# zkemail/zk-email-verify

Measured on NVIDIA H100. Metric: EmailVerifier proofs/sec (witness+prove), higher is better.
Workload: dtype u256 (BN254 Fr/Fq integers, 8x32-bit limbs)

## Files before the change

### zk-email-verify_b200/csrc/engine.cu

```cuda
#include "ff.cuh"
namespace zke { namespace dev { unsigned long long g_kernel_launches = 0; } }
#include "witness.cu"
#include "matvec.cu"
#include "ntt.cu"
#include "msm.cuh"
#include "fixed_base.cuh"
namespace zke { namespace dev {
ZKE_DEFINE_CONSTANT_UPLOAD(upload_constants_engine)
cudaError_t upload_constants_msm_g1(const FieldConsts*, const FieldConsts*);
cudaError_t upload_constants_msm_g2(const FieldConsts*, const FieldConsts*);
cudaError_t upload_constants_fixed_base(const FieldConsts*, const FieldConsts*);
cudaError_t upload_constants_verify(const FieldConsts*, const FieldConsts*);
cudaError_t upload_constants_registry(const FieldConsts*, const FieldConsts*);
} }

#include "../../include/zkemail_b200.h"
#include "cuda_host.hpp"
#include "engine.hpp"
#include "witness_program.hpp"
#include "binfile.hpp"
#include "ec_host.hpp"
#include "setup_host.hpp"
#include <algorithm>
#include <cstdio>
#include <cstring>
#include <atomic>
#include <memory>
#include <mutex>
#include <thread>
#include <unordered_map>

using namespace zke;

void zke::select_device(int device) {
    int n = 0;
    if (cudaGetDeviceCount(&n) != cudaSuccess || n == 0) throw std::runtime_error("no CUDA device available (this library has no CPU fallback)");
    if (device < 0 || device >= n) throw std::runtime_error("bad device index");
    CUDA_OK(cudaSetDevice(device));
    dev::FieldConsts fr, fq;
    fill_consts(fr, fr_params());
    fill_consts(fq, fq_params());
    CUDA_OK(dev::upload_constants_engine(&fr, &fq));
    CUDA_OK(dev::upload_constants_msm_g1(&fr, &fq));
    CUDA_OK(dev::upload_constants_msm_g2(&fr, &fq));
    CUDA_OK(dev::upload_constants_fixed_base(&fr, &fq));
    CUDA_OK(dev::upload_constants_verify(&fr, &fq));
    CUDA_OK(dev::upload_constants_registry(&fr, &fq));
    CUDA_OK(dev::configure_witness_kernel());
}

namespace {

template <class F>
std::vector<AffineH<F>> window_table(const AffineH<F>& gen) {
    std::vector<AffineH<F>> t(32 * 256, AffineH<F>::inf());
    JacobianH<F> base = JacobianH<F>::from_affine(gen);
    for (int w = 0; w < 32; ++w) {
        JacobianH<F> acc = JacobianH<F>::inf();
        for (int d = 1; d < 256; ++d) {
            acc = acc.add(base);
            t[w * 256 + d] = acc.to_affine();
        }
        for (int k = 0; k < 8; ++k) base = base.dbl();
    }
    return t;
}

std::vector<U256> to_standard(const std::vector<Fr>& v) {
    std::vector<U256> out(v.size());
    const unsigned T = std::max(1u, std::min(16u, std::thread::hardware_concurrency()));
    std::vector<std::thread> th;
    for (unsigned t = 0; t < T; ++t)
        th.emplace_back([&, t]() { for (size_t i = v.size() * t / T; i < v.size() * (t + 1) / T; ++i) out[i] = v[i].to_u256(); });
    for (auto& x : th) x.join();
    return out;
}

}

struct zke_zkey {
    uint32_t n_vars = 0, n_public = 0, log_n = 0;
    int device = 0;
    bool toy = false;
    bool delta_one = false;
    G1AffineH alpha1, beta1, delta1;
    G2AffineH beta2, gamma2, delta2;
    std::vector<G1AffineH> ic;
    DevBuf A, B1, B2, C, H;
    int h_levels = 1;
    dev::MsmConfig cfg_h;
    bool has_coefs = false;
    std::vector<uint32_t> a_ptr, a_var, a_coef, b_ptr, b_var, b_coef;
    std::vector<U256> coefs;
};

struct zke_ctx {
    const zke_circuit* circuit = nullptr;
    const zke_zkey* zkey = nullptr;
    int device = 0;
    uint32_t max_batch = 0;
    uint32_t n_vars = 0, n_public = 0, n_inputs = 0;
    cudaStream_t stream = nullptr;
    DevBuf ops, iter_hdr, lc_terms, aux, coop, coef_r, small_inv;
    std::vector<uint32_t> coef_word;
    std::vector<uint32_t> iter_info;
    DevBuf a_ptr, a_terms, b_ptr, b_terms, c_ptr, c_terms;
    dev::DevProgram prog;
    dev::DevR1cs r1cs;
    DevBuf tw_fwd, tw_inv, coset_scale;
    dev::NttTables ntt;
    size_t stride = 0;
    DevBuf inputs, check_flag;
    uint32_t inputs_resident = 0;
    struct Slot {
        bool allocated = false, busy = false;
        DevBuf w_all, inputs, results, first_bad;
        uint8_t* results_host = nullptr;
        uint8_t* publics_host = nullptr;
        std::vector<cudaEvent_t> done;
        cudaEvent_t witness_done = nullptr;
        uint32_t loaded = 0;
        uint32_t batch = 0;
        std::vector<uint8_t> rs;
    };
    Slot slots[2];
    uint64_t n_submitted = 0, n_collected = 0;
    int shard_rank = -1, shard_world = 0, shard_log_g = 0, shard_stage = 0;
    struct Lane { cudaStream_t st = nullptr, heavy = nullptr; cudaEvent_t ev[6] = {}; DevBuf va, vb, vc, vd, msm_ws; };
    Lane lanes[ZKE_MAX_LANES];
    int n_lanes = 1, lanes_alloc = 0;
    int finish_threads = 4;
    dev::MsmConfig cfg_w, cfg_h;
    bool split_streams = true;
    std::vector<uint32_t> bad_host;
    bool profile = false;
    std::vector<cudaEvent_t> ev_pool;
    size_t ev_used = 0;
    struct Span { int stage; size_t e0, e1; };
    std::vector<Span> spans;
    double stage_ms[ZKE_N_STAGES] = {0};
    uint64_t stage_count[ZKE_N_STAGES] = {0};
    cudaEvent_t ev(size_t* idx) {
        if (ev_used == ev_pool.size()) { cudaEvent_t e; cudaEventCreate(&e); ev_pool.push_back(e); }
        *idx = ev_used;
        return ev_pool[ev_used++];
    }
    size_t mark(cudaStream_t st) { size_t i; cudaEventRecord(ev(&i), st); return i; }
    size_t mark() { return mark(stream); }
    void collect() {
        for (auto& s : spans) {
            float ms = 0;
            if (cudaEventElapsedTime(&ms, ev_pool[s.e0], ev_pool[s.e1]) == cudaSuccess) { stage_ms[s.stage] += ms; stage_count[s.stage]++; }
        }
        spans.clear();
        ev_used = 0;
    }
};

static const uint32_t SETUP_SLAB = 1u << 20;
static void h_table_config(zke_zkey* zk, size_t N) {
    const char* e = getenv("ZKE_H_PRECOMP");
    const bool precomp = !(e && atoi(e) == 0);
    zk->cfg_h = dev::msm_config_full((uint32_t)N, precomp);
    zk->h_levels = precomp ? dev::msm_windows(zk->cfg_h) : 1;
}
static void build_h_levels(zke_zkey* zk, size_t N, uint8_t* scratch, cudaStream_t st) {
    for (int lvl = 1; lvl < zk->h_levels; ++lvl) {
        const uint8_t* prev = zk->H.p + (size_t)(lvl - 1) * N * sizeof(dev::G1Affine);
        uint8_t* cur = zk->H.p + (size_t)lvl * N * sizeof(dev::G1Affine);
        for (size_t off = 0; off < N; off += SETUP_SLAB) {
            uint32_t cnt = (uint32_t)std::min<size_t>(SETUP_SLAB, N - off);
            dev::scale_pow2_batch<dev::Fq>(prev + sizeof(dev::G1Affine) * off, cnt, zk->cfg_h.c, scratch, cur + sizeof(dev::G1Affine) * off, st);
        }
    }
    CHECK_LAUNCH();
    CUDA_OK(cudaStreamSynchronize(st));
}

static zke_zkey* do_setup(const zke_circuit* zc, uint64_t seed, int device) {
    select_device(device);
    const Circuit& c = zc->c;
    SetupScalars S = compute_setup_scalars(c, seed);
    std::unique_ptr<zke_zkey> zk(new zke_zkey());
    zk->n_vars = c.n_vars; zk->n_public = c.n_public(); zk->log_n = S.log_n; zk->device = device;
    zk->toy = true;
    const size_t N = (size_t)1 << S.log_n;
    const uint32_t m = c.n_vars, l = c.n_public();

    G1JacH g1 = G1JacH::from_affine(g1_generator());
    G2JacH g2 = G2JacH::from_affine(g2_generator());
    zk->alpha1 = g1.mul(S.alpha.to_u256()).to_affine();
    zk->beta1 = g1.mul(S.beta.to_u256()).to_affine();
    zk->delta1 = g1.mul(S.delta.to_u256()).to_affine();
    zk->beta2 = g2.mul(S.beta.to_u256()).to_affine();
    zk->gamma2 = g2.mul(S.gamma.to_u256()).to_affine();
    zk->delta2 = g2.mul(S.delta.to_u256()).to_affine();

    DevBuf t1, t2, scal, scratch;
    t1.upload(window_table<Fq>(g1_generator()));
    t2.upload(window_table<Fq2>(g2_generator()));
    const uint32_t SLAB = SETUP_SLAB;
// ... 479 lines not shown
    x->n_vars = cp ? cp->n_vars : zk->n_vars;
    x->n_public = cp ? cp->n_public() : zk->n_public;
    x->n_inputs = cp ? cp->n_inputs() : 0;
    int prio_least = 0, prio_greatest = 0;
    CUDA_OK(cudaDeviceGetStreamPriorityRange(&prio_least, &prio_greatest));
    CUDA_OK(cudaStreamCreateWithPriority(&x->stream, cudaStreamNonBlocking, prio_greatest));

    const std::vector<U256>& coefs = cp ? cp->coefs : zk->coefs;
    x->coef_word = coef_words(coefs);
    {
        std::vector<Fr> cr(std::max<size_t>(1, coefs.size()));
        for (size_t i = 0; i < coefs.size(); ++i) cr[i] = Fr::from_u256(coefs[i]);
        x->coef_r.upload(cr);
    }

    if (zk && cp && cp->r1cs_only && zk->has_coefs) check_key_matrices(*cp, *zk);

    if (cp && !cp->r1cs_only) upload_program(x.get(), *cp);
    upload_r1cs(x.get(), cp, zk);
    x->stride = (size_t)x->n_vars + (cp ? cp->n_temps : 0);
    x->inputs.alloc((size_t)std::max(1u, x->n_inputs) * 32 * max_batch);
    x->check_flag.alloc(8);
    x->bad_host.resize(max_batch);
    alloc_slot(x.get(), x->slots[0]);

    if (zk) {
        build_ntt_tables(x.get(), zk->log_n);
        open_lanes(x.get(), (size_t)1 << zk->log_n, prio_least, prio_greatest);
    }
    CUDA_OK(cudaDeviceSynchronize());
    return x.release();
}

static std::string assert_message(const zke_ctx* x, uint32_t email, uint32_t row) {
    std::string scope = "?";
    if (x->circuit) {
        const Circuit& c = x->circuit->c;
        if (row < c.scope_of_constraint.size()) scope = c.scopes[c.scope_of_constraint[row]];
    }
    return "Assert Failed: constraint " + std::to_string(row) + " in template " + scope + " @ email " + std::to_string(email);
}

static void require_idle(const zke_ctx* x) {
    if (x->n_submitted != x->n_collected) throw std::runtime_error("a submitted batch is still in flight: call zke_fullprove_collect first");
}

static void do_witness(zke_ctx* x, zke_ctx::Slot& S, const uint8_t* inputs, size_t batch) {
    if (!x->circuit) throw std::runtime_error("this context was opened from a .zkey alone: it has no witness program (use zke_load_witness / zke_wtns_prove)");
    const Circuit& c = x->circuit->c;
    if (c.r1cs_only) throw std::runtime_error(R1CS_NO_PROGRAM);
    if (batch == 0 || batch > x->max_batch) throw std::runtime_error("batch exceeds the context's max_batch");
    CUDA_OK(cudaSetDevice(x->device));
    const uint8_t* in_dev = x->inputs.p;
    if (inputs) {
        if (c.n_inputs()) CUDA_OK(cudaMemcpyAsync(S.inputs.p, inputs, (size_t)c.n_inputs() * 32 * batch, cudaMemcpyHostToDevice, x->stream));
        in_dev = S.inputs.p;
    } else if (x->inputs_resident < batch) {
        throw std::runtime_error("inputs == NULL but no (or too few) inputs are resident: call zke_upload_inputs first");
    }
    size_t p0 = 0;
    if (x->profile) p0 = x->mark();
    if (const char* tp = getenv("ZKE_WITNESS_TRACE")) {
        DevBuf tr;
        tr.alloc(8 * ((size_t)x->prog.n_iters + 1));
        dev::DevProgram P = x->prog;
        P.trace = (unsigned long long*)tr.p;
        dev::launch_witness(P, S.w_all.p, x->stride, in_dev, (uint32_t)batch, x->stream);
        CUDA_OK(cudaStreamSynchronize(x->stream));
        std::vector<unsigned long long> h(x->prog.n_iters);
        CUDA_OK(cudaMemcpy(h.data(), tr.p, 8 * h.size(), cudaMemcpyDeviceToHost));
        if (FILE* f = fopen(tp, "wb")) {
            fwrite(h.data(), 8, h.size(), f);
            fwrite(x->iter_info.data(), 4, x->iter_info.size(), f);
            fclose(f);
        }
    }
    dev::launch_witness(x->prog, S.w_all.p, x->stride, in_dev, (uint32_t)batch, x->stream);
    CHECK_LAUNCH();
    if (x->profile) x->spans.push_back({ZKE_STAGE_WITNESS, p0, x->mark()});
    S.loaded = (uint32_t)batch;
}

static int do_check(zke_ctx* x, zke_ctx::Slot& S, size_t batch, int32_t* status, std::string& msg) {
    CUDA_OK(cudaMemsetAsync(S.first_bad.p, 0xff, 4 * batch, x->stream));
    dev::launch_check_rows(x->r1cs, S.w_all.p, x->stride, (uint32_t)batch, (uint32_t*)S.first_bad.p, x->stream);
    CHECK_LAUNCH();
    CUDA_OK(cudaMemcpyAsync(x->bad_host.data(), S.first_bad.p, 4 * batch, cudaMemcpyDeviceToHost, x->stream));
    CUDA_OK(cudaStreamSynchronize(x->stream));
    if (x->profile) x->collect();
    int bad = 0;
    for (size_t e = 0; e < batch; ++e) {
        int32_t s = x->bad_host[e] == 0xffffffffu ? -1 : (int32_t)x->bad_host[e];
        if (status) status[e] = s;
        if (s >= 0) { if (!bad) msg = assert_message(x, (uint32_t)e, (uint32_t)s); ++bad; }
    }
    return bad;
}

static void write_fq(uint8_t* dst, const Fq& x) { U256 s = x.to_u256(); memcpy(dst, s.v, 32); }

template <class F>
static AffineH<F> finish_msm(const uint8_t* block, const dev::MsmConfig& cfg) {
    const XyzzH<F>* slots = reinterpret_cast<const XyzzH<F>*>(block);
    const int n_windows = cfg.precomputed ? 1 : (255 + cfg.c - 1) / cfg.c;
    XyzzH<F> acc = XyzzH<F>::inf();
    for (int j = n_windows - 1; j >= 0; --j) {
        if (!acc.is_inf()) for (int k = 0; k < cfg.c; ++k) acc.dbl();
        acc.add(slots[dev::MSM_ONES_SLOTS + j]);
    }
    if (cfg.classify) for (int i = 0; i < dev::MSM_ONES_SLOTS; ++i) acc.add(slots[i]);
    return acc.to_affine();
}

static void sync_lanes(zke_ctx* x) {
    cudaStreamSynchronize(x->stream);
    for (int i = 0; i < x->lanes_alloc; ++i) { cudaStreamSynchronize(x->lanes[i].st); cudaStreamSynchronize(x->lanes[i].heavy); }
}

static void enqueue_prove(zke_ctx* x, zke_ctx::Slot& S, size_t batch, const uint8_t* rs) {
    const zke_zkey* zk = x->zkey;
    if (!zk) throw std::runtime_error("context was opened without a proving key");
    if (batch == 0 || batch > S.loaded) throw std::runtime_error("no witness loaded for this batch (call zke_witness first)");
    if (rs) {
        for (size_t e = 0; e < 2 * batch; ++e) {
            U256 v;
            memcpy(v.v, rs + 32 * e, 32);
            if (u256_cmp(v, fr_params().p) >= 0) throw std::runtime_error("r / s not reduced mod the group order");
        }
        S.rs.assign(rs, rs + 64 * batch);
    } else {
        S.rs.clear();
    }
    CUDA_OK(cudaSetDevice(x->device));
    const uint32_t N = 1u << zk->log_n, m = x->n_vars, l = x->n_public;
    const bool prof = x->profile;
    const int n_lanes = prof ? 1 : x->n_lanes;
    if (const char* e = getenv("ZKE_SPLIT_STREAMS")) x->split_streams = atoi(e) != 0;
    if (l) CUDA_OK(cudaMemcpy2DAsync(S.publics_host, (size_t)l * 32, S.w_all.p + 32, x->stride * 32, (size_t)l * 32, batch, cudaMemcpyDeviceToHost, x->stream));
    CUDA_OK(cudaEventRecord(S.witness_done, x->stream));
    for (int i = 0; i < n_lanes; ++i) CUDA_OK(cudaStreamWaitEvent(x->lanes[i].st, S.witness_done, 0));
    for (size_t e = 0; e < batch; ++e) {
        zke_ctx::Lane& L = x->lanes[e % n_lanes];
        cudaStream_t st = L.st;
        const uint8_t* w = S.w_all.p + 32 * x->stride * e;
        uint8_t* res = S.results.p + (size_t)ZKE_RESULT_STRIDE * e;
        uint32_t* flag = (uint32_t*)(res + ZKE_RES_FLAG_OFF);
        size_t t0 = 0, t1 = 0;
        CUDA_OK(cudaMemsetAsync(flag, 0xff, 4, st));
        if (prof) t0 = x->mark(st);
        cudaStream_t hv = (prof || !x->split_streams) ? st : L.heavy;
        dev::launch_build_ab(x->r1cs, w, L.va.p, L.vb.p, L.vc.p, N, flag, st);
        if (prof) { t1 = x->mark(st); x->spans.push_back({ZKE_STAGE_MATVEC, t0, t1}); t0 = t1; }
        if (hv != st) { CUDA_OK(cudaEventRecord(L.ev[0], st)); CUDA_OK(cudaStreamWaitEvent(hv, L.ev[0], 0)); }
        dev::launch_intt_dif(L.va.p, x->ntt, x->coset_scale.p, hv);
        dev::launch_intt_dif(L.vb.p, x->ntt, x->coset_scale.p, hv);
        dev::launch_intt_dif(L.vc.p, x->ntt, x->coset_scale.p, hv);
        dev::launch_ntt_dit(L.va.p, x->ntt, hv);
        dev::launch_ntt_dit(L.vb.p, x->ntt, hv);
        dev::launch_ntt_dit(L.vc.p, x->ntt, hv);
        dev::launch_quotient(L.va.p, L.vb.p, L.vc.p, L.vd.p, N, hv);
        CHECK_LAUNCH();
        if (hv != st) CUDA_OK(cudaEventRecord(L.ev[1], hv));
        if (prof) { t1 = x->mark(st); x->spans.push_back({ZKE_STAGE_NTT, t0, t1}); t0 = t1; }
        uint8_t* ws_w = L.msm_ws.p;
        dev::MsmPlan<dev::Fq>::run(zk->A.p, w, m, x->cfg_w, ws_w, res + 0 * ZKE_RES_G1_BLOCK, st);
        if (prof) { t1 = x->mark(st); x->spans.push_back({ZKE_STAGE_MSM_A, t0, t1}); t0 = t1; }
        dev::MsmPlan<dev::Fq>::run(zk->B1.p, w, m, x->cfg_w, ws_w, res + 1 * ZKE_RES_G1_BLOCK, st);
        if (prof) { t1 = x->mark(st); x->spans.push_back({ZKE_STAGE_MSM_B1, t0, t1}); t0 = t1; }
        dev::MsmPlan<dev::Fq>::run(zk->C.p, w, m, x->cfg_w, ws_w, res + 2 * ZKE_RES_G1_BLOCK, st);
        if (prof) { t1 = x->mark(st); x->spans.push_back({ZKE_STAGE_MSM_C, t0, t1}); t0 = t1; }
        dev::MsmPlan<dev::Fq2>::run(zk->B2.p, w, m, x->cfg_w, ws_w, res + 4 * ZKE_RES_G1_BLOCK, st);
        CHECK_LAUNCH();
        if (prof) { t1 = x->mark(st); x->spans.push_back({ZKE_STAGE_MSM_B2, t0, t1}); t0 = t1; }
        if (hv != st) CUDA_OK(cudaStreamWaitEvent(st, L.ev[1], 0));
        {
            dev::MsmPlan<dev::Fq>::Heavy heavy{hv, L.ev[2], L.ev[3]};
            if (prof) {
                size_t i0, i1;
                cudaEvent_t evs[2];
                evs[0] = x->ev(&i0); evs[1] = x->ev(&i1);
                dev::MsmPlan<dev::Fq>::run(zk->H.p, L.vd.p, N, x->cfg_h, L.msm_ws.p, res + 3 * ZKE_RES_G1_BLOCK, st, evs, &heavy);
                x->spans.push_back({ZKE_STAGE_MSM_H_BUCKETS, i0, i1});
                t1 = x->mark(st); x->spans.push_back({ZKE_STAGE_MSM_H, t0, t1}); t0 = t1;
            } else {
                dev::MsmPlan<dev::Fq>::run(zk->H.p, L.vd.p, N, x->cfg_h, L.msm_ws.p, res + 3 * ZKE_RES_G1_BLOCK, st, nullptr, &heavy);
            }
        }
        CHECK_LAUNCH();
        CUDA_OK(cudaMemcpyAsync(S.results_host + (size_t)ZKE_RESULT_STRIDE * e, res, ZKE_RESULT_STRIDE, cudaMemcpyDeviceToHost, st));
        CUDA_OK(cudaEventRecord(S.done[e], st));
    }
    S.batch = (uint32_t)batch;
}

static int finish_prove(zke_ctx* x, zke_ctx::Slot& S, uint8_t* proofs_out, uint8_t* publics_out, int32_t* status, std::string& msg) {
    const zke_zkey* zk = x->zkey;
    const size_t batch = S.batch;
    const uint32_t l = x->n_public;
    const G1JacH alpha1 = G1JacH::from_affine(zk->alpha1), beta1 = G1JacH::from_affine(zk->beta1), delta1 = G1JacH::from_affine(zk->delta1);
    const G2JacH beta2 = G2JacH::from_affine(zk->beta2), delta2 = G2JacH::from_affine(zk->delta2);
    std::vector<int32_t> st_local(batch, -1);
    std::string first_error;
    std::mutex err_mutex;
    auto one = [&](size_t e) {
        CUDA_OK(cudaEventSynchronize(S.done[e]));
        const uint8_t* res = S.results_host + (size_t)ZKE_RESULT_STRIDE * e;
        uint32_t flag;
        memcpy(&flag, res + ZKE_RES_FLAG_OFF, 4);
        const int32_t s = flag == 0xffffffffu ? -1 : (int32_t)flag;
        st_local[e] = s;
        uint8_t* out = proofs_out + 256 * e;
        if (s >= 0) { memset(out, 0, 256); return; }
        U256 r, sc;
        if (!S.rs.empty()) { memcpy(r.v, S.rs.data() + 64 * e, 32); memcpy(sc.v, S.rs.data() + 64 * e + 32, 32); }
        else { random_scalar(r); random_scalar(sc); }
        G1AffineH ma = finish_msm<Fq>(res + 0 * ZKE_RES_G1_BLOCK, x->cfg_w);
        G1AffineH mb1 = finish_msm<Fq>(res + 1 * ZKE_RES_G1_BLOCK, x->cfg_w);
        G1AffineH mc = finish_msm<Fq>(res + 2 * ZKE_RES_G1_BLOCK, x->cfg_w);
        G1AffineH mh = finish_msm<Fq>(res + 3 * ZKE_RES_G1_BLOCK, x->cfg_h);
        G2AffineH mb2 = finish_msm<Fq2>(res + 4 * ZKE_RES_G1_BLOCK, x->cfg_w);
        G1JacH pa = alpha1.add(G1JacH::from_affine(ma)).add(delta1.mul(r));
        G2JacH pb2 = beta2.add(G2JacH::from_affine(mb2)).add(delta2.mul(sc));
        G1JacH pb1 = beta1.add(G1JacH::from_affine(mb1)).add(delta1.mul(sc));
        U256 rs_prod = (Fr::from_u256(r) * Fr::from_u256(sc)).to_u256();
        G1JacH pc = G1JacH::from_affine(mc).add(G1JacH::from_affine(mh)).add(pa.mul(sc)).add(pb1.mul(r)).add(delta1.mul(rs_prod).neg());
        G1AffineH A = pa.to_affine(), C = pc.to_affine();
        G2AffineH B = pb2.to_affine();
        write_fq(out + 0, A.x); write_fq(out + 32, A.y);
        write_fq(out + 64, B.x.c0); write_fq(out + 96, B.x.c1); write_fq(out + 128, B.y.c0); write_fq(out + 160, B.y.c1);
        write_fq(out + 192, C.x); write_fq(out + 224, C.y);
    };
    const int T = (int)std::max<size_t>(1, std::min<size_t>((size_t)x->finish_threads, batch));
    std::atomic<size_t> next{0};
    auto worker = [&]() {
        try {
            cudaSetDevice(x->device);
            for (;;) {
                const size_t e = next.fetch_add(1);
                if (e >= batch) break;
                one(e);
            }
        } catch (const std::exception& ex) {
            std::lock_guard<std::mutex> lock(err_mutex);
            if (first_error.empty()) first_error = ex.what();
        }
    };
    if (T == 1) worker();
    else {
        std::vector<std::thread> th;
        for (int t = 0; t < T; ++t) th.emplace_back(worker);
        for (auto& t : th) t.join();
    }
    if (x->profile) { sync_lanes(x); x->collect(); }
    if (!first_error.empty()) { sync_lanes(x); throw std::runtime_error(first_error); }
    int bad = 0;
    for (size_t e = 0; e < batch; ++e) {
        if (status) status[e] = st_local[e];
        if (st_local[e] >= 0) { if (!bad) msg = assert_message(x, (uint32_t)e, (uint32_t)st_local[e]); ++bad; }
    }
    if (publics_out && l) memcpy(publics_out, S.publics_host, (size_t)l * 32 * batch);
    return bad;
}

static int do_prove(zke_ctx* x, zke_ctx::Slot& S, size_t batch, const uint8_t* rs, uint8_t* proofs_out, uint8_t* publics_out, int32_t* status, std::string& msg) {
    try {
        enqueue_prove(x, S, batch, rs);
    } catch (...) {
        sync_lanes(x);
        throw;
    }
    return finish_prove(x, S, proofs_out, publics_out, status, msg);
}

static const uint8_t* parse_wtns(const uint8_t* b, size_t len, uint32_t expect_vars) {
    if (!b || len < 12 || memcmp(b, "wtns", 4) != 0) throw std::runtime_error("not a .wtns file (bad magic)");
    std::vector<BinSection> secs;
    try { secs = binfile_sections(b, len, ".wtns"); }
    catch (const std::runtime_error&) { throw std::runtime_error("truncated .wtns"); }
    const uint8_t *s1 = nullptr, *s2 = nullptr;
    size_t n1 = 0, n2 = 0;
    for (const BinSection& s : secs) {
        if (s.type == 1) { s1 = s.view.p; n1 = s.view.n; }
        if (s.type == 2) { s2 = s.view.p; n2 = s.view.n; }
    }
    if (!s1 || !s2 || n1 < 40) throw std::runtime_error(".wtns sections missing");
    if (rd32(s1) != 32 || memcmp(s1 + 4, fr_params().p.v, 32) != 0) throw std::runtime_error(".wtns is not over the BN254 scalar field");
    const uint32_t n = rd32(s1 + 36);
    if (n != expect_vars) throw std::runtime_error(".wtns has " + std::to_string(n) + " values, the key expects " + std::to_string(expect_vars));
    if (n2 != (size_t)n * 32) throw std::runtime_error(".wtns data section has the wrong size");
    return s2;
}

static void load_witness(zke_ctx* x, zke_ctx::Slot& S, const uint8_t* wtns, size_t batch) {
    if (batch == 0 || batch > x->max_batch) throw std::runtime_error("batch exceeds the context's max_batch");
    CUDA_OK(cudaSetDevice(x->device));
    const size_t m = x->n_vars;
    CUDA_OK(cudaMemcpy2DAsync(S.w_all.p, x->stride * 32, wtns, m * 32, m * 32, batch, cudaMemcpyHostToDevice, x->stream));
    CUDA_OK(cudaMemsetAsync(x->check_flag.p, 0, 8, x->stream));
    dev::launch_check_witness(S.w_all.p, x->stride, (uint32_t)m, (uint32_t)batch, (uint32_t*)x->check_flag.p, x->stream);
    CHECK_LAUNCH();
    uint32_t flags[2] = {0, 0};
    CUDA_OK(cudaMemcpyAsync(flags, x->check_flag.p, 8, cudaMemcpyDeviceToHost, x->stream));
    CUDA_OK(cudaStreamSynchronize(x->stream));
    S.loaded = 0;
    if (flags[0]) throw std::runtime_error("witness value not reduced mod r");
    if (flags[1]) throw std::runtime_error("witness[0] must be 1");
    S.loaded = (uint32_t)batch;
}

static void shard_geometry(const zke_ctx* x, int& log_m, int& log_cols, uint32_t& col0) {
    log_m = (int)x->zkey->log_n - x->shard_log_g;
    log_cols = log_m - x->shard_log_g;
    col0 = (uint32_t)x->shard_rank << log_cols;
// ... 448 lines not shown
```

### zk-email-verify_b200/csrc/ntt.cu

```cuda
#include "device_engine.cuh"
#include "ntt.cuh"
#include <cstdlib>
#include <type_traits>

namespace zke {
namespace dev {

template <bool SHOUP>
struct Twid {
    Fr w, wq;
    static constexpr uint64_t STRIDE = SHOUP ? 64 : 32;
    __device__ __forceinline__ void load(const uint8_t* base, uint64_t idx) {
        w = Fr::load(base + STRIDE * idx);
        if (SHOUP) wq = Fr::load(base + STRIDE * idx + 32);
    }
    __device__ __forceinline__ Fr mul(const Fr& x) const { return SHOUP ? Fr::mul_shoup(x, w.v, wq.v) : x * w; }
};

static const int MAX_TILE_LOG = 10;

struct Planar {
    uint32_t* sm;
    int tile;
    __device__ __forceinline__ Fr get(int e) const { Fr r; for (int i = 0; i < 8; ++i) r.v[i] = sm[i * tile + e]; return r; }
// ... 112 lines not shown
    auto tw_idx = [&](int st, uint32_t j0) -> uint64_t {
        const uint32_t idx0 = gidx(j0, l);
        return (uint64_t)(idx0 & ((1u << st) - 1)) << (log_n - 1 - st);
    };
    Twid<SHOUP> w_next;
    w_next.load(tw, tw_idx(stage_of(0), j0_of(stage_of(0))));
    __syncthreads();
#pragma unroll
    for (int step = 0; step < K; ++step) {
        const int st = stage_of(step);
        const uint32_t j0 = j0_of(st);
        const uint32_t e0 = sidx(j0, l), e1 = sidx(j0 + (1u << (st - s_lo)), l);
        const Twid<SHOUP> w = w_next;
        if (step + 1 < K) w_next.load(tw, tw_idx(stage_of(step + 1), j0_of(stage_of(step + 1))));
        const Fr u = sget(e0), v = sget(e1);
        const bool trivial = !STRIDED && st == 0;
        if (DIF) {
            sput(e0, u + v);
            sput(e1, trivial ? (u - v) : w.mul(u - v));
        } else {
            const Fr x = trivial ? v : w.mul(v);
            sput(e0, u + x);
            sput(e1, u - x);
        }
        __syncthreads();
    }
#pragma unroll
    for (int r = 0; r < 2; ++r) {
        const uint32_t e = threadIdx.x + r * 512;
        const uint32_t j = STRIDED ? (e >> L_LOG) : (e & (J - 1)), l2 = STRIDED ? (e & (L - 1)) : (e >> K);
        const uint32_t g = gidx(j, l2);
        if (scale) {
            Twid<SHOUP> sc;
            sc.load(scale, g);
            sc.mul(sget(e)).store(data + 32ull * g);
        } else {
            uint4* dst = reinterpret_cast<uint4*>(data + 32ull * g);
            dst[0] = plane0[e];
            dst[1] = plane1[e];
        }
    }
}

template <bool DIF, int K, bool STRIDED, bool SHOUP>
__global__ void __launch_bounds__(128, 3)
ntt_pass_r8_kernel(uint8_t* __restrict__ data, const uint8_t* __restrict__ tw, const uint8_t* __restrict__ scale,
                   int log_n, int s_lo_arg) {
    const int s_lo = STRIDED ? s_lo_arg : 0;
    constexpr int TILE_LOG = 10, TILE = 1 << TILE_LOG, J = 1 << K, L_LOG = TILE_LOG - K, L = 1 << L_LOG;
    constexpr int SM = TILE + TILE / 8;
    __shared__ uint4 plane0[SM], plane1[SM];
    const int s_hi = s_lo + K - 1;
    const uint32_t bid = blockIdx.x;
    uint32_t hi = 0, lo_base = 0;
    if constexpr (STRIDED) {
        const uint32_t lo_blocks_log = s_lo - L_LOG;
        lo_base = (bid & ((1u << lo_blocks_log) - 1)) << L_LOG;
        hi = bid >> lo_blocks_log;
    }
    auto gidx = [&](uint32_t j, uint32_t l) -> uint32_t {
        return STRIDED ? ((hi << (s_hi + 1)) | (j << s_lo) | (lo_base + l)) : ((((bid << L_LOG) + l) << K) | j);
    };
    auto pad = [](uint32_t e) -> uint32_t { return e + (e >> 3); };
    auto sget = [&](uint32_t e) -> Fr {
        const uint4 a = plane0[pad(e)], b = plane1[pad(e)];
        Fr r; r.v[0] = a.x; r.v[1] = a.y; r.v[2] = a.z; r.v[3] = a.w; r.v[4] = b.x; r.v[5] = b.y; r.v[6] = b.z; r.v[7] = b.w;
        return r;
    };
    auto sput = [&](uint32_t e, const Fr& x) {
        plane0[pad(e)] = make_uint4(x.v[0], x.v[1], x.v[2], x.v[3]);
        plane1[pad(e)] = make_uint4(x.v[4], x.v[5], x.v[6], x.v[7]);
    };
#pragma unroll
    for (int r = 0; r < 8; ++r) {
        const uint32_t e = threadIdx.x + r * 128;
        const uint32_t j = STRIDED ? (e >> L_LOG) : (e & (J - 1)), l = STRIDED ? (e & (L - 1)) : (e >> K);
        const uint4* src = reinterpret_cast<const uint4*>(data + 32ull * gidx(j, l));
        plane0[pad(e)] = src[0];
        plane1[pad(e)] = src[1];
    }
    __syncthreads();
    auto round = [&](auto b_tag, auto r_tag) {
        constexpr int B = decltype(b_tag)::value, R = decltype(r_tag)::value, NR = 1 << R;
        constexpr int BP = STRIDED ? B + L_LOG : B;
        constexpr int ITEMS = TILE >> R;
#pragma unroll 1
        for (uint32_t u = threadIdx.x; u < ITEMS; u += 128) {
            const uint32_t base = (u & ((1u << BP) - 1)) | ((u >> BP) << (BP + R));
            const uint32_t j = STRIDED ? (base >> L_LOG) : (base & (J - 1)), l = STRIDED ? (base & (L - 1)) : (base >> K);
            Fr x[NR];
#pragma unroll
            for (int r = 0; r < NR; ++r) x[r] = sget(base + ((uint32_t)r << BP));
#pragma unroll
            for (int qq = 0; qq < R; ++qq) {
                const int q = DIF ? (R - 1 - qq) : qq;
                const int st = s_lo + B + q;
                const bool trivial = !STRIDED && B + q == 0;
                Twid<SHOUP> w[NR / 2];
                if (!trivial) {
#pragma unroll
                    for (int p = 0; p < NR / 2; ++p) {
                        const int r0 = ((p >> q) << (q + 1)) | (p & ((1 << q) - 1));
                        const uint32_t idx0 = gidx(j | ((uint32_t)r0 << B), l);
                        w[p].load(tw, (uint64_t)(idx0 & ((1u << st) - 1)) << (log_n - 1 - st));
                    }
                }
#pragma unroll
                for (int p = 0; p < NR / 2; ++p) {
                    const int r0 = ((p >> q) << (q + 1)) | (p & ((1 << q) - 1)), r1 = r0 | (1 << q);
                    const Fr a = x[r0], b = x[r1];
                    if (DIF) {
                        x[r0] = a + b;
                        x[r1] = trivial ? (a - b) : w[p].mul(a - b);
                    } else {
                        const Fr y = trivial ? b : w[p].mul(b);
                        x[r0] = a + y;
                        x[r1] = a - y;
                    }
                }
            }
#pragma unroll
            for (int r = 0; r < NR; ++r) sput(base + ((uint32_t)r << BP), x[r]);
        }
        __syncthreads();
    };
    using std::integral_constant;
    constexpr int R0 = K >= 3 ? 3 : K, K1 = K - R0, R1 = K1 >= 3 ? 3 : K1, R2 = K1 - R1;
    if (DIF) {
        round(integral_constant<int, K - R0>{}, integral_constant<int, R0>{});
        if constexpr (R1 > 0) round(integral_constant<int, K - R0 - R1>{}, integral_constant<int, R1>{});
        if constexpr (R2 > 0) round(integral_constant<int, 0>{}, integral_constant<int, R2>{});
    } else {
        round(integral_constant<int, 0>{}, integral_constant<int, R0>{});
        if constexpr (R1 > 0) round(integral_constant<int, R0>{}, integral_constant<int, R1>{});
        if constexpr (R2 > 0) round(integral_constant<int, R0 + R1>{}, integral_constant<int, R2>{});
    }
#pragma unroll
    for (int r = 0; r < 8; ++r) {
        const uint32_t e = threadIdx.x + r * 128;
        const uint32_t j = STRIDED ? (e >> L_LOG) : (e & (J - 1)), l2 = STRIDED ? (e & (L - 1)) : (e >> K);
        const uint32_t g = gidx(j, l2);
        if (scale) {
            Twid<SHOUP> sc;
            sc.load(scale, g);
            sc.mul(sget(e)).store(data + 32ull * g);
        } else {
            uint4* dst = reinterpret_cast<uint4*>(data + 32ull * g);
            dst[0] = plane0[pad(e)];
            dst[1] = plane1[pad(e)];
        }
    }
}

template <bool DIF, bool SHOUP>
static bool launch_fast(uint8_t* data, const uint8_t* tw, const uint8_t* scale, int log_n, int s_lo, int s_hi, cudaStream_t st, int log_tw) {
    if (log_n < 10) return false;
    const int k = s_hi - s_lo + 1;
    const uint32_t blocks = 1u << (log_n - 10);
    const bool strided = s_lo > 0;
    if (strided && s_lo < 10 - k) return false;
    static const bool r8 = getenv("ZKE_NTT_R8") && atoi(getenv("ZKE_NTT_R8")) != 0;
#define ZKE_NTT_CASE(KK)                                                                                            \
    case KK:                                                                                                       \
        if (r8) {                                                                                                  \
            if (strided) ntt_pass_r8_kernel<DIF, KK, true, SHOUP><<<blocks, 128, 0, st>>>(data, tw, scale, log_tw, s_lo);  \
            else ntt_pass_r8_kernel<DIF, KK, false, SHOUP><<<blocks, 128, 0, st>>>(data, tw, scale, log_tw, s_lo);         \
        } else if (strided) ntt_pass_fast_kernel<DIF, KK, true, SHOUP><<<blocks, 512, 0, st>>>(data, tw, scale, log_tw, s_lo); \
        else ntt_pass_fast_kernel<DIF, KK, false, SHOUP><<<blocks, 512, 0, st>>>(data, tw, scale, log_tw, s_lo);            \
        return true;
    switch (k) {
        ZKE_NTT_CASE(4) ZKE_NTT_CASE(5) ZKE_NTT_CASE(6) ZKE_NTT_CASE(7) ZKE_NTT_CASE(8)
        default: return false;
    }
#undef ZKE_NTT_CASE
}

static void plan(int log_n, int* lo, int* hi, int* n_pass) {
    int passes = (log_n + 7) / 8;
    int base = log_n / passes, extra = log_n % passes;
    int top = log_n - 1;
    for (int p = 0; p < passes; ++p) {
        int k = base + (p < extra ? 1 : 0);
        hi[p] = top;
        lo[p] = top - k + 1;
        top -= k;
    }
    *n_pass = passes;
}

static void intt_dif_impl(uint8_t* data, const NttTables& T, int log_local, const uint8_t* scale_bitrev, cudaStream_t st) {
    int lo[4], hi[4], np;
    plan(log_local, lo, hi, &np);
    ZKE_COUNT_LAUNCH(np);
    const int tile_log = log_local < MAX_TILE_LOG ? log_local : MAX_TILE_LOG;
    const uint32_t blocks = 1u << (log_local - tile_log);
    for (int p = 0; p < np; ++p) {
        const uint8_t* sc = p == np - 1 ? scale_bitrev : nullptr;
        if (T.shoup ? launch_fast<true, true>(data, T.tw_inv, sc, log_local, lo[p], hi[p], st, T.log_n)
                    : launch_fast<true, false>(data, T.tw_inv, sc, log_local, lo[p], hi[p], st, T.log_n)) continue;
        if (T.shoup) ntt_pass_kernel<true, true><<<blocks, 1 << (tile_log - 1), 32u << tile_log, st>>>(data, T.tw_inv, sc, T.log_n, lo[p], hi[p], tile_log);
        else ntt_pass_kernel<true, false><<<blocks, 1 << (tile_log - 1), 32u << tile_log, st>>>(data, T.tw_inv, sc, T.log_n, lo[p], hi[p], tile_log);
    }
}
static void ntt_dit_impl(uint8_t* data, const NttTables& T, int log_local, cudaStream_t st) {
    int lo[4], hi[4], np;
    plan(log_local, lo, hi, &np);
    ZKE_COUNT_LAUNCH(np);
    const int tile_log = log_local < MAX_TILE_LOG ? log_local : MAX_TILE_LOG;
    const uint32_t blocks = 1u << (log_local - tile_log);
    for (int p = np - 1; p >= 0; --p) {
        if (T.shoup ? launch_fast<false, true>(data, T.tw_fwd, nullptr, log_local, lo[p], hi[p], st, T.log_n)
                    : launch_fast<false, false>(data, T.tw_fwd, nullptr, log_local, lo[p], hi[p], st, T.log_n)) continue;
        if (T.shoup) ntt_pass_kernel<false, true><<<blocks, 1 << (tile_log - 1), 32u << tile_log, st>>>(data, T.tw_fwd, nullptr, T.log_n, lo[p], hi[p], tile_log);
        else ntt_pass_kernel<false, false><<<blocks, 1 << (tile_log - 1), 32u << tile_log, st>>>(data, T.tw_fwd, nullptr, T.log_n, lo[p], hi[p], tile_log);
    }
}
void launch_intt_dif(uint8_t* data, const NttTables& T, const uint8_t* scale_bitrev, cudaStream_t st) { intt_dif_impl(data, T, T.log_n, scale_bitrev, st); }
void launch_ntt_dit(uint8_t* data, const NttTables& T, cudaStream_t st) { ntt_dit_impl(data, T, T.log_n, st); }
void launch_intt_dif_block(uint8_t* block, const NttTables& T, int log_local, const uint8_t* scale_block, cudaStream_t st) { intt_dif_impl(block, T, log_local, scale_block, st); }
void launch_ntt_dit_block(uint8_t* block, const NttTables& T, int log_local, cudaStream_t st) { ntt_dit_impl(block, T, log_local, st); }

template <bool DIF, int LOGG, bool SHOUP>
__global__ void __launch_bounds__(128)
ntt_cross_kernel(uint8_t* __restrict__ data, const uint8_t* __restrict__ tw, int log_n, uint32_t col0, uint32_t n_cols) {
    constexpr int G = 1 << LOGG;
    const uint32_t t = blockIdx.x * blockDim.x + threadIdx.x;
    if (t >= n_cols) return;
    const int log_m = log_n - LOGG;
    const uint32_t j = col0 + t;
    Fr x[G];
#pragma unroll
    for (int g = 0; g < G; ++g) x[g] = Fr::load(data + 32ull * (((uint32_t)g << log_m) + j));
#pragma unroll
    for (int step = 0; step < LOGG; ++step) {
        const int sb = DIF ? (LOGG - 1 - step) : step;
        const int st = log_m + sb;
#pragma unroll
        for (int g0 = 0; g0 < G; ++g0) {
            if (g0 & (1 << sb)) continue;
            const int g1 = g0 | (1 << sb);
            const uint32_t idx0 = ((uint32_t)g0 << log_m) + j;
            const uint64_t tw_i = (uint64_t)(idx0 & ((1u << st) - 1)) << (log_n - 1 - st);
            Twid<SHOUP> w;
            w.load(tw, tw_i);
            const Fr u = x[g0], v = x[g1];
            if (DIF) {
                x[g0] = u + v;
                x[g1] = w.mul(u - v);
            } else {
                const Fr y = w.mul(v);
                x[g0] = u + y;
                x[g1] = u - y;
            }
        }
    }
#pragma unroll
    for (int g = 0; g < G; ++g) x[g].store(data + 32ull * (((uint32_t)g << log_m) + j));
}
template <bool DIF, bool SHOUP>
static void launch_cross(uint8_t* data, const uint8_t* tw, int log_n, int log_g, uint32_t col0, uint32_t n_cols, cudaStream_t st) {
    const uint32_t blocks = (n_cols + 127) / 128;
    switch (log_g) {
        case 1: ntt_cross_kernel<DIF, 1, SHOUP><<<blocks, 128, 0, st>>>(data, tw, log_n, col0, n_cols); break;
        case 2: ntt_cross_kernel<DIF, 2, SHOUP><<<blocks, 128, 0, st>>>(data, tw, log_n, col0, n_cols); break;
        case 3: ntt_cross_kernel<DIF, 3, SHOUP><<<blocks, 128, 0, st>>>(data, tw, log_n, col0, n_cols); break;
        default: break;
    }
    ZKE_COUNT_LAUNCH(1);
}
void launch_intt_cross(uint8_t* data, const NttTables& T, int log_g, uint32_t col0, uint32_t n_cols, cudaStream_t st) {
    if (T.shoup) launch_cross<true, true>(data, T.tw_inv, T.log_n, log_g, col0, n_cols, st);
    else launch_cross<true, false>(data, T.tw_inv, T.log_n, log_g, col0, n_cols, st);
}
void launch_ntt_cross(uint8_t* data, const NttTables& T, int log_g, uint32_t col0, uint32_t n_cols, cudaStream_t st) {
    if (T.shoup) launch_cross<false, true>(data, T.tw_fwd, T.log_n, log_g, col0, n_cols, st);
    else launch_cross<false, false>(data, T.tw_fwd, T.log_n, log_g, col0, n_cols, st);
}

__global__ void hadamard_kernel(const uint8_t* __restrict__ a, const uint8_t* __restrict__ b, uint8_t* __restrict__ c, uint32_t n) {
    uint32_t i = blockIdx.x * blockDim.x + threadIdx.x;
    if (i >= n) return;
    (Fr::load(a + 32ull * i) * Fr::load(b + 32ull * i)).store(c + 32ull * i);
}
void launch_hadamard(const uint8_t* a, const uint8_t* b, uint8_t* c, uint32_t n, cudaStream_t st) {
    hadamard_kernel<<<(n + 255) / 256, 256, 0, st>>>(a, b, c, n);
    ZKE_COUNT_LAUNCH(1);
}

__global__ void quotient_kernel(const uint8_t* __restrict__ a, const uint8_t* __restrict__ b, const uint8_t* __restrict__ c,
                                uint8_t* __restrict__ d, uint32_t n) {
    uint32_t i = blockIdx.x * blockDim.x + threadIdx.x;
    if (i >= n) return;
    Fr x = Fr::load(a + 32ull * i) * Fr::load(b + 32ull * i) - Fr::load(c + 32ull * i);
    x.from_mont().store(d + 32ull * i);
}
void launch_quotient(const uint8_t* a, const uint8_t* b, const uint8_t* c, uint8_t* d, uint32_t n, cudaStream_t st) {
    quotient_kernel<<<(n + 255) / 256, 256, 0, st>>>(a, b, c, d, n);
    ZKE_COUNT_LAUNCH(1);
}
__global__ void quotient_cols_kernel(const uint8_t* __restrict__ a, const uint8_t* __restrict__ b, const uint8_t* __restrict__ c,
                                     uint8_t* __restrict__ d, uint32_t n_threads, int log_m, int log_cols, uint32_t col0) {
    const uint32_t t = blockIdx.x * blockDim.x + threadIdx.x;
    if (t >= n_threads) return;
    const uint32_t i = ((t >> log_cols) << log_m) + col0 + (t & ((1u << log_cols) - 1));
    Fr x = Fr::load(a + 32ull * i) * Fr::load(b + 32ull * i) - Fr::load(c + 32ull * i);
    x.from_mont().store(d + 32ull * i);
}
void launch_quotient_cols(const uint8_t* a, const uint8_t* b, const uint8_t* c, uint8_t* d, int log_n, int log_g, uint32_t col0, uint32_t n_cols_log, cudaStream_t st) {
    const uint32_t n_threads = (1u << log_g) << n_cols_log;
    quotient_cols_kernel<<<(n_threads + 255) / 256, 256, 0, st>>>(a, b, c, d, n_threads, log_n - log_g, (int)n_cols_log, col0);
    ZKE_COUNT_LAUNCH(1);
}

}
}
```

### zk-email-verify_b200/csrc/ntt.cuh

```cuda
#pragma once
#include <cstdint>
#include <cuda_runtime.h>

namespace zke {
namespace dev {

struct NttTables {
    const uint8_t* tw_fwd;
    const uint8_t* tw_inv;
    int log_n;
    bool shoup;
};

void launch_intt_dif(uint8_t* data, const NttTables& T, const uint8_t* scale_bitrev, cudaStream_t st);
void launch_ntt_dit(uint8_t* data, const NttTables& T, cudaStream_t st);
void launch_intt_dif_block(uint8_t* block, const NttTables& T, int log_local, const uint8_t* scale_block, cudaStream_t st);
void launch_ntt_dit_block(uint8_t* block, const NttTables& T, int log_local, cudaStream_t st);
void launch_intt_cross(uint8_t* data, const NttTables& T, int log_g, uint32_t col0, uint32_t n_cols, cudaStream_t st);
void launch_ntt_cross(uint8_t* data, const NttTables& T, int log_g, uint32_t col0, uint32_t n_cols, cudaStream_t st);
void launch_quotient_cols(const uint8_t* a, const uint8_t* b, const uint8_t* c, uint8_t* d, int log_n, int log_g, uint32_t col0, uint32_t n_cols_log, cudaStream_t st);
void launch_hadamard(const uint8_t* a, const uint8_t* b, uint8_t* c, uint32_t n, cudaStream_t st);
void launch_quotient(const uint8_t* a, const uint8_t* b, const uint8_t* c, uint8_t* d, uint32_t n, cudaStream_t st);

}
}
```

Baseline: 47.79.

## Batch three NTT vectors per pass and fuse quotient into final forward pass

Adds a kernel that runs each NTT pass on the A, B and C vectors together in one launch, with a 512-thread block holding three 1024-element tiles in 96KB of shared memory. Each twiddle load is shared by all three vectors, and the launch count for the NTT stage drops to a third. The final forward pass computes a*b-c, converts it out of Montgomery form and writes it directly, so the separate quotient kernel and its extra read of the three vectors go away. The large shared footprint limits occupancy to about two blocks per SM. The fused path only uses non-Shoup twiddles and otherwise falls back to the old code.

```diff
diff --git a/zk-email-verify_b200/csrc/engine.cu b/zk-email-verify_b200/csrc/engine.cu
--- a/zk-email-verify_b200/csrc/engine.cu
+++ b/zk-email-verify_b200/csrc/engine.cu
@@ -47,6 +47,7 @@
     CUDA_OK(dev::upload_constants_verify(&fr, &fq));
     CUDA_OK(dev::upload_constants_registry(&fr, &fq));
     CUDA_OK(dev::configure_witness_kernel());
+    CUDA_OK(dev::configure_ntt_kernels());
 }
 
 namespace {
@@ -832,13 +833,8 @@
         dev::launch_build_ab(x->r1cs, w, L.va.p, L.vb.p, L.vc.p, N, flag, st);
         if (prof) { t1 = x->mark(st); x->spans.push_back({ZKE_STAGE_MATVEC, t0, t1}); t0 = t1; }
         if (hv != st) { CUDA_OK(cudaEventRecord(L.ev[0], st)); CUDA_OK(cudaStreamWaitEvent(hv, L.ev[0], 0)); }
-        dev::launch_intt_dif(L.va.p, x->ntt, x->coset_scale.p, hv);
-        dev::launch_intt_dif(L.vb.p, x->ntt, x->coset_scale.p, hv);
-        dev::launch_intt_dif(L.vc.p, x->ntt, x->coset_scale.p, hv);
-        dev::launch_ntt_dit(L.va.p, x->ntt, hv);
-        dev::launch_ntt_dit(L.vb.p, x->ntt, hv);
-        dev::launch_ntt_dit(L.vc.p, x->ntt, hv);
-        dev::launch_quotient(L.va.p, L.vb.p, L.vc.p, L.vd.p, N, hv);
+        dev::launch_intt_dif3(L.va.p, L.vb.p, L.vc.p, x->ntt, x->coset_scale.p, hv);
+        dev::launch_ntt_dit3_quotient(L.va.p, L.vb.p, L.vc.p, L.vd.p, x->ntt, hv);
         CHECK_LAUNCH();
         if (hv != st) CUDA_OK(cudaEventRecord(L.ev[1], hv));
         if (prof) { t1 = x->mark(st); x->spans.push_back({ZKE_STAGE_NTT, t0, t1}); t0 = t1; }
diff --git a/zk-email-verify_b200/csrc/ntt.cu b/zk-email-verify_b200/csrc/ntt.cu
--- a/zk-email-verify_b200/csrc/ntt.cu
+++ b/zk-email-verify_b200/csrc/ntt.cu
@@ -288,6 +288,125 @@
     }
 }
 
+static constexpr int NTT3_THREADS = 512;
+static constexpr int NTT3_SMEM = 3 * 2 * 1024 * (int)sizeof(uint4);
+
+template <bool DIF, int K, bool STRIDED>
+__global__ void __launch_bounds__(NTT3_THREADS, 2)
+ntt3_pass_kernel(uint8_t* __restrict__ va, uint8_t* __restrict__ vb, uint8_t* __restrict__ vc, const uint8_t* __restrict__ tw,
+                 const uint8_t* __restrict__ scale, uint8_t* __restrict__ quot, int log_n, int s_lo_arg) {
+    const int s_lo = STRIDED ? s_lo_arg : 0;
+    constexpr int TILE_LOG = 10, TILE = 1 << TILE_LOG, J = 1 << K, L_LOG = TILE_LOG - K, L = 1 << L_LOG;
+    constexpr int BF = TILE / 2 / NTT3_THREADS, PER = TILE / NTT3_THREADS;
+    extern __shared__ uint4 ntt3_smem[];
+    uint8_t* const vec[3] = {va, vb, vc};
+    const int s_hi = s_lo + K - 1;
+    const uint32_t bid = blockIdx.x;
+    uint32_t hi = 0, lo_base = 0;
+    if constexpr (STRIDED) {
+        const uint32_t lo_blocks_log = s_lo - L_LOG;
+        lo_base = (bid & ((1u << lo_blocks_log) - 1)) << L_LOG;
+        hi = bid >> lo_blocks_log;
+    }
+    auto gidx = [&](uint32_t j, uint32_t l) -> uint32_t {
+        return STRIDED ? ((hi << (s_hi + 1)) | (j << s_lo) | (lo_base + l)) : ((((bid << L_LOG) + l) << K) | j);
+    };
+    auto sidx = [&](uint32_t j, uint32_t l) -> uint32_t { return STRIDED ? ((j << L_LOG) + l) : ((l << K) + j); };
+    auto sget = [&](int v, uint32_t e) -> Fr {
+        const uint4 a = ntt3_smem[2 * v * TILE + e], b = ntt3_smem[(2 * v + 1) * TILE + e];
+        Fr r; r.v[0] = a.x; r.v[1] = a.y; r.v[2] = a.z; r.v[3] = a.w; r.v[4] = b.x; r.v[5] = b.y; r.v[6] = b.z; r.v[7] = b.w;
+        return r;
+    };
+    auto sput = [&](int v, uint32_t e, const Fr& x) {
+        ntt3_smem[2 * v * TILE + e] = make_uint4(x.v[0], x.v[1], x.v[2], x.v[3]);
+        ntt3_smem[(2 * v + 1) * TILE + e] = make_uint4(x.v[4], x.v[5], x.v[6], x.v[7]);
+    };
+#pragma unroll
+    for (int v = 0; v < 3; ++v) {
+#pragma unroll
+        for (int r = 0; r < PER; ++r) {
+            const uint32_t e = threadIdx.x + r * NTT3_THREADS;
+            const uint32_t j = STRIDED ? (e >> L_LOG) : (e & (J - 1)), l = STRIDED ? (e & (L - 1)) : (e >> K);
+            const uint4* src = reinterpret_cast<const uint4*>(vec[v] + 32ull * gidx(j, l));
+            ntt3_smem[2 * v * TILE + e] = src[0];
+            ntt3_smem[(2 * v + 1) * TILE + e] = src[1];
+        }
+    }
+    uint32_t l[BF], jj[BF];
+#pragma unroll
+    for (int i = 0; i < BF; ++i) {
+        const uint32_t t = threadIdx.x + i * NTT3_THREADS;
+        l[i] = STRIDED ? (t & (L - 1)) : (t >> (K - 1));
+        jj[i] = STRIDED ? (t >> L_LOG) : (t & (J / 2 - 1));
+    }
+    auto stage_of = [&](int step) { return DIF ? (s_hi - step) : (s_lo + step); };
+    auto j0_of = [&](int st, uint32_t jj_i) -> uint32_t {
+        const uint32_t hb = st - s_lo;
+        return ((jj_i >> hb) << (hb + 1)) | (jj_i & ((1u << hb) - 1));
+    };
+    auto tw_idx = [&](int st, int i) -> uint64_t {
+        const uint32_t idx0 = gidx(j0_of(st, jj[i]), l[i]);
+        return (uint64_t)(idx0 & ((1u << st) - 1)) << (log_n - 1 - st);
+    };
+    auto trivial = [&](int step) { return !STRIDED && stage_of(step) == 0; };
+    Twid<false> w_next[BF];
+#pragma unroll
+    for (int i = 0; i < BF; ++i)
+        if (!trivial(0)) w_next[i].load(tw, tw_idx(stage_of(0), i));
+    __syncthreads();
+#pragma unroll
+    for (int step = 0; step < K; ++step) {
+        const int st = stage_of(step);
+#pragma unroll
+        for (int i = 0; i < BF; ++i) {
+            const uint32_t j0 = j0_of(st, jj[i]);
+            const uint32_t e0 = sidx(j0, l[i]), e1 = sidx(j0 + (1u << (st - s_lo)), l[i]);
+            const Twid<false> w = w_next[i];
+            if (step + 1 < K && !trivial(step + 1)) w_next[i].load(tw, tw_idx(stage_of(step + 1), i));
+#pragma unroll
+            for (int v = 0; v < 3; ++v) {
+                const Fr u = sget(v, e0), x = sget(v, e1);
+                if (DIF) {
+                    sput(v, e0, u + x);
+                    sput(v, e1, trivial(step) ? (u - x) : w.mul(u - x));
+                } else {
+                    const Fr y = trivial(step) ? x : w.mul(x);
+                    sput(v, e0, u + y);
+                    sput(v, e1, u - y);
+                }
+            }
+        }
+        __syncthreads();
+    }
+#pragma unroll
+    for (int r = 0; r < PER; ++r) {
+        const uint32_t e = threadIdx.x + r * NTT3_THREADS;
+        const uint32_t j = STRIDED ? (e >> L_LOG) : (e & (J - 1)), l2 = STRIDED ? (e & (L - 1)) : (e >> K);
+        const uint32_t g = gidx(j, l2);
+        if (quot) {
+            const Fr d = sget(0, e) * sget(1, e) - sget(2, e);
+            d.from_mont().store(quot + 32ull * g);
+        } else if (scale) {
+            Twid<false> sc;
+            sc.load(scale, g);
+#pragma unroll
+            for (int v = 0; v < 3; ++v) sc.mul(sget(v, e)).store(vec[v] + 32ull * g);
+        } else {
+#pragma unroll
+            for (int v = 0; v < 3; ++v) {
+                uint4* dst = reinterpret_cast<uint4*>(vec[v] + 32ull * g);
+                dst[0] = ntt3_smem[2 * v * TILE + e];
+                dst[1] = ntt3_smem[(2 * v + 1) * TILE + e];
+            }
+        }
+    }
+}
+
+static bool ntt_r8_requested() {
+    static const bool r8 = getenv("ZKE_NTT_R8") && atoi(getenv("ZKE_NTT_R8")) != 0;
+    return r8;
+}
+
 template <bool DIF, bool SHOUP>
 static bool launch_fast(uint8_t* data, const uint8_t* tw, const uint8_t* scale, int log_n, int s_lo, int s_hi, cudaStream_t st, int log_tw) {
     if (log_n < 10) return false;
@@ -295,7 +414,7 @@
     const uint32_t blocks = 1u << (log_n - 10);
     const bool strided = s_lo > 0;
     if (strided && s_lo < 10 - k) return false;
-    static const bool r8 = getenv("ZKE_NTT_R8") && atoi(getenv("ZKE_NTT_R8")) != 0;
+    const bool r8 = ntt_r8_requested();
 #define ZKE_NTT_CASE(KK)                                                                                            \
     case KK:                                                                                                       \
         if (r8) {                                                                                                  \
@@ -355,6 +474,67 @@
 void launch_ntt_dit(uint8_t* data, const NttTables& T, cudaStream_t st) { ntt_dit_impl(data, T, T.log_n, st); }
 void launch_intt_dif_block(uint8_t* block, const NttTables& T, int log_local, const uint8_t* scale_block, cudaStream_t st) { intt_dif_impl(block, T, log_local, scale_block, st); }
 void launch_ntt_dit_block(uint8_t* block, const NttTables& T, int log_local, cudaStream_t st) { ntt_dit_impl(block, T, log_local, st); }
+
+static bool ntt3_takes(const NttTables& T) {
+    if (T.shoup || ntt_r8_requested() || T.log_n < MAX_TILE_LOG) return false;
+    int lo[4], hi[4], np;
+    plan(T.log_n, lo, hi, &np);
+    for (int p = 0; p < np; ++p) {
+        const int k = hi[p] - lo[p] + 1;
+        if (k < 4 || k > 8 || (lo[p] > 0 && lo[p] < MAX_TILE_LOG - k)) return false;
+    }
+    return true;
+}
+template <bool DIF>
+static void launch_ntt3_pass(uint8_t* a, uint8_t* b, uint8_t* c, const uint8_t* tw, const uint8_t* scale, uint8_t* quot, int log_n,
+                             int s_lo, int s_hi, cudaStream_t st) {
+    const uint32_t blocks = 1u << (log_n - MAX_TILE_LOG);
+#define ZKE_NTT3_CASE(KK)                                                                                                  \
+    case KK:                                                                                                             \
+        if (s_lo > 0) ntt3_pass_kernel<DIF, KK, true><<<blocks, NTT3_THREADS, NTT3_SMEM, st>>>(a, b, c, tw, scale, quot, log_n, s_lo); \
+        else ntt3_pass_kernel<DIF, KK, false><<<blocks, NTT3_THREADS, NTT3_SMEM, st>>>(a, b, c, tw, scale, quot, log_n, s_lo);         \
+        break;
+    switch (s_hi - s_lo + 1) {
+        ZKE_NTT3_CASE(4) ZKE_NTT3_CASE(5) ZKE_NTT3_CASE(6) ZKE_NTT3_CASE(7) ZKE_NTT3_CASE(8)
+        default: break;
+    }
+#undef ZKE_NTT3_CASE
+}
+void launch_intt_dif3(uint8_t* a, uint8_t* b, uint8_t* c, const NttTables& T, const uint8_t* scale_bitrev, cudaStream_t st) {
+    if (!ntt3_takes(T)) {
+        for (uint8_t* v : {a, b, c}) launch_intt_dif(v, T, scale_bitrev, st);
+        return;
+    }
+    int lo[4], hi[4], np;
+    plan(T.log_n, lo, hi, &np);
+    ZKE_COUNT_LAUNCH(np);
+    for (int p = 0; p < np; ++p)
+        launch_ntt3_pass<true>(a, b, c, T.tw_inv, p == np - 1 ? scale_bitrev : nullptr, nullptr, T.log_n, lo[p], hi[p], st);
+}
+void launch_ntt_dit3_quotient(uint8_t* a, uint8_t* b, uint8_t* c, uint8_t* d, const NttTables& T, cudaStream_t st) {
+    if (!ntt3_takes(T)) {
+        for (uint8_t* v : {a, b, c}) launch_ntt_dit(v, T, st);
+        launch_quotient(a, b, c, d, 1u << T.log_n, st);
+        return;
+    }
+    int lo[4], hi[4], np;
+    plan(T.log_n, lo, hi, &np);
+    ZKE_COUNT_LAUNCH(np);
+    for (int p = np - 1; p >= 0; --p)
+        launch_ntt3_pass<false>(a, b, c, T.tw_fwd, nullptr, p == 0 ? d : nullptr, T.log_n, lo[p], hi[p], st);
+}
+cudaError_t configure_ntt_kernels() {
+#define ZKE_NTT3_K(KK) ntt3_pass_kernel<true, KK, false>, ntt3_pass_kernel<true, KK, true>, ntt3_pass_kernel<false, KK, false>, ntt3_pass_kernel<false, KK, true>,
+    void (*const kernels[])(uint8_t*, uint8_t*, uint8_t*, const uint8_t*, const uint8_t*, uint8_t*, int, int) = {
+        ZKE_NTT3_K(4) ZKE_NTT3_K(5) ZKE_NTT3_K(6) ZKE_NTT3_K(7) ZKE_NTT3_K(8)};
+#undef ZKE_NTT3_K
+    for (auto k : kernels) {
+        cudaError_t e = cudaFuncSetAttribute(k, cudaFuncAttributeMaxDynamicSharedMemorySize, NTT3_SMEM);
+        if (e == cudaSuccess) e = cudaFuncSetAttribute(k, cudaFuncAttributePreferredSharedMemoryCarveout, cudaSharedmemCarveoutMaxShared);
+        if (e != cudaSuccess) return e;
+    }
+    return cudaSuccess;
+}
 
 template <bool DIF, int LOGG, bool SHOUP>
 __global__ void __launch_bounds__(128)
diff --git a/zk-email-verify_b200/csrc/ntt.cuh b/zk-email-verify_b200/csrc/ntt.cuh
--- a/zk-email-verify_b200/csrc/ntt.cuh
+++ b/zk-email-verify_b200/csrc/ntt.cuh
@@ -19,6 +19,9 @@
 void launch_intt_cross(uint8_t* data, const NttTables& T, int log_g, uint32_t col0, uint32_t n_cols, cudaStream_t st);
 void launch_ntt_cross(uint8_t* data, const NttTables& T, int log_g, uint32_t col0, uint32_t n_cols, cudaStream_t st);
 void launch_quotient_cols(const uint8_t* a, const uint8_t* b, const uint8_t* c, uint8_t* d, int log_n, int log_g, uint32_t col0, uint32_t n_cols_log, cudaStream_t st);
+void launch_intt_dif3(uint8_t* a, uint8_t* b, uint8_t* c, const NttTables& T, const uint8_t* scale_bitrev, cudaStream_t st);
+void launch_ntt_dit3_quotient(uint8_t* a, uint8_t* b, uint8_t* c, uint8_t* d, const NttTables& T, cudaStream_t st);
+cudaError_t configure_ntt_kernels();
 void launch_hadamard(const uint8_t* a, const uint8_t* b, uint8_t* c, uint32_t n, cudaStream_t st);
 void launch_quotient(const uint8_t* a, const uint8_t* b, const uint8_t* c, uint8_t* d, uint32_t n, cudaStream_t st);
 
```

Result: faster. 48.79, median of 6 (+2.1%).
